# Lightbrite88/Argon_Monte_Carlo

Hardware: AMD Instinct MI355X
Metric: particle-steps/sec (higher is better)
Workload: dtype f64; 1 GPU; cube_1e5; geometry=cube, n_particles=100000, n_per_gpu=100000, parallelism=single GPU

## Files before the change

### argon_monte_carlo_amd/csrc/amc_grid.hip

```cpp
#include <stdlib.h>

#include "amc_grid_dev.h"

#define AMC_CR2_INFLATE (1.0 + 1.0e-9)

__global__ __launch_bounds__(256) void k_bin_lists(const double *__restrict__ x, const double *__restrict__ y,
                                                   const double *__restrict__ z, long long n, amc_grid G, amc_lists B,
                                                   amc_dev_counters *cnt, amc_ovl V)
{
    const long long p = (long long)blockIdx.x * blockDim.x + threadIdx.x;
    if (p >= n) return;
    if (V.skip_epoch && (unsigned int)(V.adj_head[p] >> 32) == V.skip_epoch) return;
    bool outside = false;
    amc_list_insert(G, B, (int)p, x[p], y[p], z[p], &outside);
    if (outside) atomicOr(&cnt->flags, 8ULL);
}

struct amc_adj {
    unsigned long long *head;
    int4 *rec;
    int4 *sd;
    int4 *sl_meta;
    int *sl_hits, *ev_gen;
    unsigned int epoch;
    unsigned long long *mark;
};

AMC_DEV int amc_push_candidate(int a, int b, int max_cand, amc_dev_counters *cnt, const amc_adj &D)
{
    const unsigned int k = atomicAdd(&cnt->cand_count, 1u);
    if (k < (unsigned)max_cand) {
        const int hi = a > b ? a : b, lo = a > b ? b : a;
        int4 r;
        r.x = hi; r.y = lo; r.z = -1; r.w = -1;
        if (D.head) {
            const unsigned long long mine = ((unsigned long long)D.epoch << 32) | (unsigned long long)k;
            const unsigned long long oi = atomicExch(&D.head[hi], mine), oj = atomicExch(&D.head[lo], mine);
            r.z = ((unsigned int)(oi >> 32) == D.epoch) ? (int)(unsigned int)(oi & 0xffffffffULL) : -1;
            r.w = ((unsigned int)(oj >> 32) == D.epoch) ? (int)(unsigned int)(oj & 0xffffffffULL) : -1;
            auto mark = [&](int kd) {
                const unsigned long long old = atomicExch(&D.mark[kd], mine);
                if ((unsigned int)(old >> 32) == D.epoch) D.mark[kd] = ((unsigned long long)D.epoch << 32) | AMC_MARK_MULTI;
            };
            if (r.z >= 0) mark(r.z);
            if (r.w >= 0) mark(r.w);
        }
        D.rec[k] = r;
        D.sd[k] = make_int4(-1, -1, 0, 0);
        if (D.head) {
            D.sl_meta[2 * k] = make_int4(-1, 2 * (int)k, 0, 0);
            D.sl_meta[2 * k + 1] = make_int4(-1, 2 * (int)k + 1, 0, 0);
            atomicAnd(&D.sl_hits[2 * k], 0);
            atomicAnd(&D.sl_hits[2 * k + 1], 0);
            *(int4 *)&D.ev_gen[4 * k] = make_int4(0, 0, 0, 0);
        }
        return (int)k;
    }
    atomicOr(&cnt->flags, 1ULL);
    return -1;
}

AMC_DEV void amc_detect_node(const amc_grid &G, const amc_lists &B, int node, double cr2i, double cr_probe, int max_cand,
                             amc_dev_counters *cnt, const amc_adj &D, const int *od_stall = nullptr, int od_tick = 0)
{
    const int stalled = od_stall ? *od_stall : 0;
    amc_rec me_r = B.rec[node];
    const int live = (B.node_of && node < B.n) ? B.node_of[node] : node;
    if (stalled && od_tick > stalled) return;
    if (me_r.x != me_r.x) {
        if (live == node) return;
        node = live;
        me_r = B.rec[node];
        if (me_r.x != me_r.x) return;
    }
    const int me_p = amc_node_particle(B, node);
    double3 me;
    amc_rec_pos(G, me_r, me.x, me.y, me.z);
    auto found_pair = [&](int q) { amc_push_candidate(me_p, amc_node_particle(B, q), max_cand, cnt, D); };
    int q[9];
    q[0] = amc_rec_next(me_r);
    {
        int ocx, ocy, ocz;
        amc_grid_coords(G, me.x, me.y, me.z, ocx, ocy, ocz);
        const int c_own = amc_grid_cell(G, ocx, ocy, ocz, nullptr);
        int c_lo[4], c_hi[4];
        const int nc = amc_grid_box_ranges(G, me.x, me.y, me.z, cr_probe, c_lo, c_hi);
        int cell[8];
#pragma unroll
        for (int k = 0; k < 4; k++)
#pragma unroll
            for (int t = 0; t < 2; t++) {
                const int c = c_lo[k < nc ? k : 0] + t;
                cell[2 * k + t] = (k < nc && c <= c_hi[k < nc ? k : 0] && c < c_own) ? c : -1;
            }
        unsigned long long hv[8];
#pragma unroll
        for (int e = 0; e < 8; e++) hv[e] = (cell[e] >= 0) ? B.head[cell[e]] : 0ULL;
#pragma unroll
        for (int e = 0; e < 8; e++)
            q[1 + e] = (cell[e] >= 0 && (unsigned int)(hv[e] >> 32) == B.epoch) ? (int)(unsigned int)(hv[e] & 0xffffffffULL) : -1;
    }
    for (;;) {
        bool live = false;
#pragma unroll
        for (int e = 0; e < 9; e++) live |= q[e] >= 0;
        if (!live) break;
        amc_rec o[9];
#pragma unroll
        for (int e = 0; e < 9; e++)
            if (q[e] >= 0) o[e] = B.rec[q[e]];
#pragma unroll
        for (int e = 0; e < 9; e++)
            if (q[e] >= 0) {
                double ox, oy, oz;
                amc_rec_pos(G, o[e], ox, oy, oz);
                const double ex = ox - me.x, ey = oy - me.y, ez = oz - me.z;
                if (ex * ex + ey * ey + ez * ez < cr2i) found_pair(q[e]);
                q[e] = amc_rec_next(o[e]);
            }
    }
}

#ifndef AMC_DETECT_MINW
#define AMC_DETECT_MINW 4
#endif
__global__ __launch_bounds__(256, AMC_DETECT_MINW) void k_detect_lists(amc_grid G, amc_lists B, long long n, double cr2i, double cr_probe,
                                                      int max_cand, amc_dev_counters *cnt, amc_adj D, const int *extra_count,
                                                      int max_extra, const int *od_stall, int od_tick, int *wctl_rearm)
{
    const long long nb = (n + blockDim.x - 1) / blockDim.x;
    if ((long long)blockIdx.x < nb) {
        const long long p = (long long)blockIdx.x * blockDim.x + threadIdx.x;
        if (p < n) amc_detect_node(G, B, (int)p, cr2i, cr_probe, max_cand, cnt, D, od_stall, od_tick);
        if (wctl_rearm && p == 0 && !(*od_stall && od_tick > *od_stall)) {
            amc_resolve_ctl *wc = (amc_resolve_ctl *)wctl_rearm;
            for (int b = 0; b < 16; b++) wctl_rearm[32 + b] = 0;
            wc->nslots = 0; wc->nhist = 0; wc->nedges = 0; wc->nfp = 0; wc->ovf = 0; wc->dirty = 0; wc->nclusters = 0;
            wc->changed = 0; wc->active = 0; wc->cur_round = 1;
        }
        return;
    }
    if (!extra_count) return;
    int ne = *extra_count;
    if (ne > max_extra) ne = max_extra;
    const int stride = (int)((gridDim.x - nb) * blockDim.x);
    for (int e = (int)((blockIdx.x - nb) * blockDim.x + threadIdx.x); e < ne; e += stride)
        amc_detect_node(G, B, (int)n + e, cr2i, cr_probe, max_cand, cnt, D, od_stall, od_tick);
}

__global__ __launch_bounds__(256) void k_detect_own(amc_grid G, amc_lists B, long long lo, long long hi, double cr2i,
                                                    double cr_probe, int *__restrict__ out, int cap, amc_dev_counters *cnt)
{
    const long long p = lo + (long long)blockIdx.x * blockDim.x + threadIdx.x;
    if (p >= hi) return;
    amc_rec me_r = B.rec[p];
    const int live = B.node_of ? B.node_of[p] : (int)p;
    if (me_r.x != me_r.x) {
        if (live == (int)p) return;
        me_r = B.rec[live];
        if (me_r.x != me_r.x) return;
    }
    double3 me;
    amc_rec_pos(G, me_r, me.x, me.y, me.z);
    int c_lo[4], c_hi[4];
    const int nc = amc_grid_box_ranges(G, me.x, me.y, me.z, cr_probe, c_lo, c_hi);
    int q[8];
    unsigned long long hv[8];
#pragma unroll
    for (int k = 0; k < 4; k++)
#pragma unroll
        for (int t = 0; t < 2; t++) {
            const int c = c_lo[k < nc ? k : 0] + t;
            const bool on = k < nc && c <= c_hi[k < nc ? k : 0];
            hv[2 * k + t] = on ? B.head[c] : 0ULL;
            q[2 * k + t] = on ? 0 : -1;
        }
#pragma unroll
    for (int e = 0; e < 8; e++)
        q[e] = (q[e] == 0 && (unsigned int)(hv[e] >> 32) == B.epoch) ? (int)(unsigned int)(hv[e] & 0xffffffffULL) : -1;
    for (;;) {
        bool live = false;
#pragma unroll
        for (int e = 0; e < 8; e++) live |= q[e] >= 0;
        if (!live) break;
        amc_rec o[8];
#pragma unroll
        for (int e = 0; e < 8; e++)
            if (q[e] >= 0) o[e] = B.rec[q[e]];
#pragma unroll
        for (int e = 0; e < 8; e++)
            if (q[e] >= 0) {
                double ox, oy, oz;
                amc_rec_pos(G, o[e], ox, oy, oz);
                const double ex = ox - me.x, ey = oy - me.y, ez = oz - me.z;
                const int pq = amc_node_particle(B, q[e]);
                if (pq < (int)p && ex * ex + ey * ey + ez * ez < cr2i) {
                    const int k = atomicAdd(&out[0], 1);
                    if (k < cap) { out[2 + 2 * k] = (int)p; out[3 + 2 * k] = pq; }
                    else atomicOr(&cnt->flags, 1ULL);
                }
                q[e] = amc_rec_next(o[e]);
            }
    }
}

__global__ __launch_bounds__(256) void k_ingest_candidates(const int *__restrict__ blocks, int world, int block_ints, int cap,
                                                           int max_cand, amc_dev_counters *cnt, amc_adj D, int *__restrict__ own)
{
    const int gtid = blockIdx.x * blockDim.x + threadIdx.x, gstride = gridDim.x * blockDim.x;
    for (int r = 0; r < world; r++) {
        const int *b = blocks + (size_t)r * block_ints;
        int nr = b[0];
        if (nr > cap) {
            nr = cap;
            if (gtid == 0) atomicOr(&cnt->flags, 1ULL);
        }
        for (int k = gtid; k < nr; k += gstride) amc_push_candidate(b[2 + 2 * k], b[3 + 2 * k], max_cand, cnt, D);
    }
    if (gtid == 0) own[0] = 0;
}

#define AP_T 256
__global__ __launch_bounds__(AP_T) void k_detect_allpairs(const double *__restrict__ x, const double *__restrict__ y,
                                                          const double *__restrict__ z, int n, int ntiles, double cr2i,
                                                          int max_cand, amc_dev_counters *cnt, amc_adj D)
{
    int bi = (int)((sqrt(8.0 * (double)blockIdx.x + 1.0) - 1.0) * 0.5);
    while ((long long)(bi + 1) * (bi + 2) / 2 <= (long long)blockIdx.x) bi++;
    while ((long long)bi * (bi + 1) / 2 > (long long)blockIdx.x) bi--;
    const int bj = (int)(blockIdx.x - (long long)bi * (bi + 1) / 2);
    if (bi >= ntiles) return;
    __shared__ double tx[AP_T], ty[AP_T], tz[AP_T];
    const int j0 = bj * AP_T;
    const int jj = j0 + threadIdx.x;
    tx[threadIdx.x] = (jj < n) ? x[jj] : 0.0;
    ty[threadIdx.x] = (jj < n) ? y[jj] : 0.0;
    tz[threadIdx.x] = (jj < n) ? z[jj] : 0.0;
    __syncthreads();
    const int i = bi * AP_T + threadIdx.x;
    if (i >= n) return;
    const double xi = x[i], yi = y[i], zi = z[i];
    int jmax = n - j0;
    if (jmax > AP_T) jmax = AP_T;
    if (bi == bj && jmax > (int)threadIdx.x) jmax = threadIdx.x;
#pragma unroll 4
    for (int k = 0; k < jmax; k++) {
        const double ex = tx[k] - xi, ey = ty[k] - yi, ez = tz[k] - zi;
        const double d2 = fma(ez, ez, fma(ey, ey, ex * ex));
        if (d2 < cr2i) amc_push_candidate(i, j0 + k, max_cand, cnt, D);
    }
}

hipError_t amc_launch_bin(amc_ctx *c)
{
    if (c->allpairs || c->n <= 0) return hipSuccess;
    const long long n = c->n;
    c->B.epoch++;
    c->step.lists_age = -1;
    amc_prof_begin(c, AMC_K_BIN_COUNT);
    amc_ovl V;
    V.adj_head = nullptr; V.skip_epoch = 0;
    AMC_LAUNCH(c, k_bin_lists, dim3((unsigned)((n + 255) / 256)), dim3(256), c->S.x, c->S.y, c->S.z, n,
                       c->G, c->B, c->d_cnt, V);
    amc_prof_end(c);
    return hipGetLastError();
}

hipError_t amc_launch_bin_ovl(amc_ctx *c, int to, unsigned int skip_epoch, hipStream_t stream)
{
    const long long n = c->n;
    amc_ovl V;
    V.adj_head = c->W.adj_head; V.skip_epoch = skip_epoch;
    amc_prof_begin(c, AMC_K_BIN_COUNT);
    AMC_LAUNCH_ON(c, stream, k_bin_lists, dim3((unsigned)((n + 255) / 256)), dim3(256), c->S_buf[to].x, c->S_buf[to].y, c->S_buf[to].z, n,
                  c->G, c->B_buf[to], c->d_cnt, V);
    amc_prof_end(c);
    return hipGetLastError();
}

#define AP2_T 1024
#define AP2_R 4
#define AP2_THREADS (AP2_T / AP2_R)
#define AP2_CHUNK 8
__global__ __launch_bounds__(AP2_THREADS) void k_detect_allpairs_tiled(const double *__restrict__ x, const double *__restrict__ y,
                                                               const double *__restrict__ z, int n, int ntiles, double thr,
                                                               double ox, double oy, double oz,
                                                               int max_cand, amc_dev_counters *cnt, amc_adj D)
{
    int bi = (int)((sqrt(8.0 * (double)blockIdx.x + 1.0) - 1.0) * 0.5);
    while ((long long)(bi + 1) * (bi + 2) / 2 <= (long long)blockIdx.x) bi++;
    while ((long long)bi * (bi + 1) / 2 > (long long)blockIdx.x) bi--;
    const int bj = (int)(blockIdx.x - (long long)bi * (bi + 1) / 2);
    if (bi >= ntiles) return;
    __shared__ double tx[AP2_T], ty[AP2_T], tz[AP2_T], tn[AP2_T];
    const int j0 = bj * AP2_T;
    for (int t = threadIdx.x; t < AP2_T; t += AP2_THREADS) {
        const int jj = j0 + t;
        const bool in = jj < n;
        const double X = in ? x[jj] - ox : 0.0, Y = in ? y[jj] - oy : 0.0, Z = in ? z[jj] - oz : 0.0;
        tx[t] = X; ty[t] = Y; tz[t] = Z;
        tn[t] = in ? fma(Z, Z, fma(Y, Y, X * X)) : 1.0e300;
    }
    __syncthreads();
    int ii[AP2_R];
    double ax[AP2_R], ay[AP2_R], az[AP2_R], ti[AP2_R];
#pragma unroll
    for (int r = 0; r < AP2_R; r++) {
        ii[r] = bi * AP2_T + r * AP2_THREADS + (int)threadIdx.x;
        const bool in = ii[r] < n;
        const double X = in ? x[ii[r]] - ox : 0.0, Y = in ? y[ii[r]] - oy : 0.0, Z = in ? z[ii[r]] - oz : 0.0;
        ax[r] = -2.0 * X; ay[r] = -2.0 * Y; az[r] = -2.0 * Z;
        ti[r] = in ? thr - fma(Z, Z, fma(Y, Y, X * X)) : -1.0e300;
    }
    const bool diag = bi == bj;
    for (int k0 = 0; k0 < AP2_T; k0 += AP2_CHUNK) {
        bool any = false;
#pragma unroll
        for (int u = 0; u < AP2_CHUNK; u++) {
            const double jx = tx[k0 + u], jy = ty[k0 + u], jz = tz[k0 + u], jn = tn[k0 + u];
#pragma unroll
            for (int r = 0; r < AP2_R; r++) any |= fma(az[r], jz, fma(ay[r], jy, fma(ax[r], jx, jn))) < ti[r];
        }
        if (any) {
            for (int u = 0; u < AP2_CHUNK; u++) {
                const int j = j0 + k0 + u;
                const double jx = tx[k0 + u], jy = ty[k0 + u], jz = tz[k0 + u], jn = tn[k0 + u];
#pragma unroll
                for (int r = 0; r < AP2_R; r++)
                    if (fma(az[r], jz, fma(ay[r], jy, fma(ax[r], jx, jn))) < ti[r] && (diag ? j < ii[r] : true))
                        amc_push_candidate(ii[r], j, max_cand, cnt, D);
            }
        }
    }
}

static unsigned int next_sweep_epoch(unsigned int epoch)
{
    epoch = (epoch + 1u) & 0x3fffffffu;
    return epoch ? epoch : 1u;
}

hipError_t amc_launch_detect(amc_ctx *c)
{
    const long long n = c->n;
    if (n <= 0) return hipSuccess;
    const double cr2i = c->allpairs || c->detect_ap ? c->P.collision_range * c->P.collision_range * AMC_CR2_INFLATE : c->G.cr2_probe;
    amc_adj D;
    c->step.sweep_epoch = next_sweep_epoch(c->step.sweep_epoch);
    c->step.plan_split = !c->allpairs && !(c->h_host_ncand && *c->h_host_ncand <= c->plan_small);
    D.head = c->allpairs ? nullptr : c->W.adj_head; D.rec = c->W.cand4; D.sd = c->W.cand_s; D.epoch = c->step.sweep_epoch;
    D.sl_meta = c->W.sl_meta; D.sl_hits = c->W.sl_hits; D.ev_gen = c->W.ev_gen; D.mark = c->W.cand_mark;
    amc_prof_begin(c, AMC_K_DETECT);
    if (c->detect_ap) {
        if (n >= 16 * AP2_T && c->G.ncells > 0) {
            const int ntiles = (int)((n + AP2_T - 1) / AP2_T);
            const long long nblocks = (long long)ntiles * (ntiles + 1) / 2;
            const double ex = c->G.gx * c->G.h, ey = c->G.gy * c->G.h, ez = c->G.gz * c->G.h;
            const double thr = cr2i + 64.0 * 1.1102230246251565e-16 * (ex * ex + ey * ey + ez * ez);
            AMC_LAUNCH(c, k_detect_allpairs_tiled, dim3((unsigned)nblocks), dim3(AP2_THREADS), c->S.x, c->S.y,
                               c->S.z, (int)n, ntiles, thr, c->G.x0, c->G.y0, c->G.z0, c->W.max_cand, c->d_cnt, D);
        } else {
            const int ntiles = (int)((n + AP_T - 1) / AP_T);
            const long long nblocks = (long long)ntiles * (ntiles + 1) / 2;
            if (nblocks > 0)
                AMC_LAUNCH(c, k_detect_allpairs, dim3((unsigned)nblocks), dim3(AP_T), c->S.x, c->S.y,
                                   c->S.z, (int)n, ntiles, cr2i, c->W.max_cand, c->d_cnt, D);
        }
    } else {
        const bool extras = c->B.extra != nullptr && c->keep_K < 2;
        const int slot = (c->B.extra == c->extra_buf[1]) ? 1 : 0;
        const int bs = c->detect_bs;
        AMC_LAUNCH(c, k_detect_lists, dim3((unsigned)((n + bs - 1) / bs) + (extras ? 4u : 0u)), dim3(bs), c->G, c->B, n, cr2i,
                   c->G.cr_probe, c->W.max_cand, c->d_cnt, D, (const int *)(extras ? c->extra_count + slot : nullptr),
                   c->max_extra, (const int *)(c->od_active ? c->d_od : nullptr), c->od_tick,
                   (c->od_active && !c->step.od_prev_ordered) ? c->W.wctl : nullptr);
    }
    amc_prof_end(c);
    return hipGetLastError();
}

hipError_t amc_launch_detect_own(amc_ctx *c)
{
    const long long cnt = c->hi - c->lo;
    amc_prof_begin(c, AMC_K_DETECT);
    if (cnt > 0)
        AMC_LAUNCH(c, k_detect_own, dim3((unsigned)((cnt + 255) / 256)), dim3(256), c->G, c->B, (long long)c->lo, (long long)c->hi,
                   c->G.cr2_probe, c->G.cr_probe, c->MG.cand_send, c->MG.cand_cap, c->d_cnt);
    amc_prof_end(c);
    return hipGetLastError();
}

hipError_t amc_launch_ingest(amc_ctx *c, int world)
{
    amc_adj D;
    c->step.sweep_epoch = next_sweep_epoch(c->step.sweep_epoch);
    c->step.plan_split = !(c->h_host_ncand && *c->h_host_ncand <= c->plan_small);
    D.head = c->W.adj_head; D.rec = c->W.cand4; D.sd = c->W.cand_s; D.epoch = c->step.sweep_epoch;
    D.sl_meta = c->W.sl_meta; D.sl_hits = c->W.sl_hits; D.ev_gen = c->W.ev_gen; D.mark = c->W.cand_mark;
    amc_prof_begin(c, AMC_K_DETECT);
    AMC_LAUNCH(c, k_ingest_candidates, dim3(16), dim3(256), (const int *)c->MG.cand_recv, world, 2 + 2 * c->MG.cand_cap, c->MG.cand_cap,
               c->W.max_cand, c->d_cnt, D, c->MG.cand_send);
    amc_prof_end(c);
    return hipGetLastError();
}
```

### argon_monte_carlo_amd/csrc/amc_internal.h

```cpp
#pragma once
#include <hip/hip_runtime.h>
#include <hip/hip_ext.h>
#include <stdint.h>

#include <string>
#include <vector>

#include "amc_device.h"

#define RS_SLOT_DOUBLES 12

struct amc_state {
    double *x, *y, *z, *vx, *vy, *vz, *d, *dx, *dy, *dz;
    double *px, *py, *pz;
    uint8_t *flag;
};

struct amc_grid {
    double x0, y0, z0, h;
    double inv_h;
    int uniform;
    int gx, gy, gz;
    int ncells;
    double cr_probe;
    double cr2_probe;
    const int *lay_lo;
    const int *lay_n;
    const int *lay_off;
};

struct amc_rec {
    float x, y, z;
    int next;
};
#define AMC_MARK_MULTI 0xffffffffu
struct amc_lists {
    unsigned long long *head;
    amc_rec *rec;
    unsigned int epoch;
    int n;
    int *extra;
    int *cell_of;
    int *node_of;
    int *wave_count;
    int wave_cap;
};
#define AMC_LIST_KEEP_DEFAULT_PORE 4
#define AMC_EXTRA_NODES(n) ((int)std::min<long long>(std::max<long long>(4096, (long long)(n) / 64), 1 << 22))

struct amc_ovl {
    const unsigned long long *adj_head;
    unsigned int skip_epoch;
};

struct amc_lazy {
    int *slot_of;
    const double *state;
    const uint8_t *moved;
    int enabled;
};

struct amc_resolve_ctl {
    int nslots, nedges, nhist, nev, dirty, changed, nhits, nfp, ovf, nclusters, ncomplex;
    int rounds, ncand, active, ok, edges_done;
    int lazy_ns, nslots0, hist_begin, cur_round;
};
struct rs_event {
    int phase, i, j, which;
    long long cell;
    int slot, pad;
    double val[4];
};
struct amc_resolve_ws {
    int4 *cand4, *cand_s;
    unsigned long long *cand_mark;
    int max_cand;
    unsigned long long *adj_head;
    int *slot_of;
    unsigned int *victim;
    int max_slots;
    int4 *sl_meta;
    int *sl_hits;
    uint8_t *sl_moved;
    double *sl_state;
    int *edge_a, *edge_b;
    int max_edges;
    double4 *hist;
    int max_hist;
    int *ov_head, *ov_next;
    int *ev_gen;
    rs_event *ev;
    int *ctl;
    int *wctl;
    int *raise_dev, *raise_host;
    int raise_tick;
    int *sl_label, *sl_tmp;
    uint8_t *sl_dirty;
    unsigned long long *sl_key;
    int *order;
    double *cw_d[10];
    int *cw_tmp, *cw_pidx, *cw_slot;
    uint8_t *cw_flag, *cw_moved;
};

struct amc_temp_handover {
    int hits_case = -1, hits_n = 0;
    int ahead_case = -1;
    std::vector<int> perm;
    int parked_case = -1, parked_n = 0;
    std::vector<int> parked_perm;
    void fresh() { hits_case = ahead_case = parked_case = -1; hits_n = parked_n = 0; perm.clear(); parked_perm.clear(); }
};

struct amc_temp_ws {
    int *idx, *count;
    double *t, *contact, *normal, *dir, *Es, *dpz, *dE;
    unsigned char *ok;
    int *h_idx, *h_count;
    double *h_contact, *h_normal, *h_dir, *h_Es, *h_dpz, *h_dE;
    void *pin;
    int cap;
    int *def_idx;
    double *def_dir, *def_Es, *def_dpz, *def_dE;
    double *h_def_Es, *h_def_dpz, *h_def_dE;
    amc_temp_handover h;
};

struct temp_dev_segments {
    int *idx, *count;
    double *t, *contact, *normal, *dir, *Es, *dpz, *dE;
    unsigned char *ok;
    int cap;
};
struct amc_temp_pass {
    amc_temp_rng g;
    temp_dev_segments D;
};
struct amc_temp_row {
    double sums[3];
    unsigned int had;
    unsigned int pad;
};
struct amc_temp_dev_ws {
    temp_dev_segments seg;
    amc_temp_row *series;
    int64_t series_cap, series_n;
    int *perm;
    int *ovf;
    amc_temp_pass *pass;
    bool fetched;
    int h_count[7];
    std::vector<int> h_idx[7];
    std::vector<double> h_dpz[7], h_dE[7];
    std::vector<unsigned char> h_ok[7];
};

struct amc_fields_grid_dev {
    int kind, n1, n2, n3, bins;
    double lo[3], hi[3], w[3];
};

// ... 251 lines not shown
```

### argon_monte_carlo_amd/csrc/amc_stream.hip

```cpp
#include <stdlib.h>
#include <string.h>

#include <algorithm>

#include "amc_commit_dev.h"
#include "amc_energised_dev.h"

struct amc_stream_counts {
    int nwall, nerr, noob, noob_pre;
};

template <int GEOM>
AMC_DEV void amc_stream_particle(amc_particle &q, const amc_params &P, const amc_out &O, double dt, int stages, int ip,
                                 double &px, double &py, double &pz, amc_stream_counts &cn)
{
    if ((stages & AMC_ST_BOUNDS_PRE) && GEOM != AMC_GEOM_CUBE)
        cn.noob_pre = amc_bounds(P, q.x, q.y, q.z, GEOM == AMC_GEOM_PORE_ENERGISED);
    if (stages & AMC_ST_DRIFT) {
        px = q.x; py = q.y; pz = q.z;
        const double sx = dt * q.vx, sy = dt * q.vy, sz = dt * q.vz;
        q.x += sx; q.y += sy; q.z += sz;
        q.d += fabs(sqrt(sx * sx + sy * sy + sz * sz));
        q.dx += fabs(sx); q.dy += fabs(sy); q.dz += fabs(sz);
    }
    if (stages & AMC_ST_WALLS) {
        if (GEOM == AMC_GEOM_CUBE) {
#define AMC_CUBE_AXIS(pos, vel, W)                                                                    \
    if (pos > W) { const double t_ = (pos - W) / vel; vel = -vel; pos = W + t_ * vel; }                \
    if (pos < 0) { const double t_ = pos / vel; vel = -vel; pos = t_ * vel; }
            AMC_CUBE_AXIS(q.x, q.vx, P.cube_x)
            AMC_CUBE_AXIS(q.y, q.vy, P.cube_y)
            AMC_CUBE_AXIS(q.z, q.vz, P.cube_z)
#undef AMC_CUBE_AXIS
        } else if (GEOM == AMC_GEOM_PORE) {
            const double zb = P.z_gap_bottom, zt = P.z_gap_top;
            const double r0 = sqrt(px * px + py * py);
            if (sqrt(q.x * q.x + q.y * q.y) > P.R_oa) {
                if (amc_side_wall(q, P.R_oa_c, true, O, 1, ip)) cn.nerr++; else cn.nwall++;
            }
            if (q.z < 0) { amc_vertical_wall(q, 0.0, O, 2, ip); cn.nwall++; }
            if (q.z > P.H) { amc_vertical_wall(q, P.H, O, 3, ip); cn.nwall++; }
            if ((pz > P.z_cold) && (q.z < P.z_cold) && (sqrt(q.x * q.x + q.y * q.y) > P.R_p)) {
                amc_vertical_wall(q, P.z_cold, O, 4, ip); cn.nwall++;
            }
            if ((pz < P.h_oa) && (q.z > P.h_oa) && (sqrt(q.x * q.x + q.y * q.y) > P.R_p)) {
                amc_vertical_wall(q, P.h_oa, O, 5, ip); cn.nwall++;
            }
            if ((pz < zt) && (pz > zb) && (r0 < P.R_g) && (sqrt(q.x * q.x + q.y * q.y) > P.R_g)) {
                if (amc_side_wall(q, P.R_g_c, true, O, 6, ip)) cn.nerr++; else cn.nwall++;
            }
            if ((r0 > P.R_p) && (q.z < zb) && (pz < zt) && (pz > zb)) {
                amc_vertical_wall(q, zb, O, 7, ip); cn.nwall++;
            }
            if ((r0 > P.R_p) && (q.z > zt) && (pz < zt) && (pz > zb)) {
                amc_vertical_wall(q, zt, O, 8, ip); cn.nwall++;
            }
            if ((r0 < P.R_p) && (sqrt(q.x * q.x + q.y * q.y) > P.R_p) &&
                (((q.z < P.z_cold) && (q.z > zt)) || ((q.z < zb) && (q.z > P.h_oa)))) {
                if (amc_side_wall(q, P.R_p_c, true, O, 9, ip)) cn.nerr++; else cn.nwall++;
            }
        } else if (GEOM == AMC_GEOM_PORE_ENERGISED) {
            if (sqrt(q.x * q.x + q.y * q.y) > P.R_oa) {
                if (amc_side_wall(q, P.R_oa_c, false, O, 1, ip)) cn.nerr++;
            }
            if (q.z < 0) { const double t_ = (q.z - 0.0) / q.vz; q.vz = -q.vz; q.z = 0.0 + t_ * q.vz; }
            if (q.z > P.H) { const double t_ = (q.z - P.H) / q.vz; q.vz = -q.vz; q.z = P.H + t_ * q.vz; }
        }
    }
    if ((stages & AMC_ST_BOUNDS) && GEOM != AMC_GEOM_CUBE)
        cn.noob = amc_bounds(P, q.x, q.y, q.z, GEOM == AMC_GEOM_PORE_ENERGISED);
}

AMC_DEV void amc_stream_count(const amc_out &O, const amc_stream_counts &cn, int bounds_slot, int ip)
{
    if (!(cn.nwall | cn.nerr | cn.noob | cn.noob_pre)) return;
    if (O.wev.count) {
        amc_wev_rec r;
        r.p = ip; r.kind = 1; r.a = cn.nwall | (cn.nerr << 16); r.b = cn.noob | (cn.noob_pre << 16);
        r.v[0] = r.v[1] = r.v[2] = r.v[3] = 0.0;
        amc_wev_append(O, r);
        return;
    }
    if (cn.nwall) atomicAdd(&O.banks[amc_bank_id()].n_wall, (unsigned long long)cn.nwall);
    if (cn.nerr) atomicAdd(&O.banks[amc_bank_id()].n_fp_errors, (unsigned long long)cn.nerr);
    if (cn.noob) atomicAdd(bounds_slot ? &O.cnt->n_oob_pp : &O.cnt->n_oob_walls, (unsigned long long)cn.noob);
    if (cn.noob_pre) atomicAdd(&O.cnt->n_oob_pp, (unsigned long long)cn.noob_pre);
}

#define AMC_LD(p) __builtin_nontemporal_load(&(p))
#define AMC_ST(p, v) __builtin_nontemporal_store((v), &(p))

template <int GEOM, int TEMP = 0>
__global__ __launch_bounds__(256) void k_stream(amc_state S, amc_state S_out, amc_params P, amc_out O, double dt, int stages,
                                                long long lo, long long hi, int keep_prior, int bounds_slot,
                                                amc_grid G, amc_lists B, int build_lists, amc_lazy L, amc_commit_args C,
                                                amc_ovl V, const amc_temp_pass *TP)
{
    const int stalled = C.od_stall ? *C.od_stall : 0;
    if (C.enabled) {
        const unsigned nstream = gridDim.x - (unsigned)C.enabled;
        if (blockIdx.x >= nstream) {
            if (stalled && C.od_tick > stalled) return;
            amc_out Oc = O;
            Oc.step = C.step;
            amc_commit_part(C, Oc, G, S, (int)((blockIdx.x - nstream) * blockDim.x + threadIdx.x), (int)(C.enabled * blockDim.x));
            return;
        }
    }
    const long long p = lo + (long long)blockIdx.x * blockDim.x + threadIdx.x;
    if (p >= hi) return;
    if (V.skip_epoch && (unsigned int)(V.adj_head[p] >> 32) == V.skip_epoch) return;
    const int wave_id = (int)(blockIdx.x * (blockDim.x >> 6) + (threadIdx.x >> 6));
    const int keep_count0 = build_lists == 3 ? B.wave_count[wave_id] : 0;
    const int keep_cell = build_lists == 3 ? B.cell_of[p] : -1, keep_node = build_lists == 3 ? B.node_of[p] : (int)p;
    amc_particle q;
    q.x = AMC_LD(S.x[p]); q.y = AMC_LD(S.y[p]); q.z = AMC_LD(S.z[p]);
    q.vx = AMC_LD(S.vx[p]); q.vy = AMC_LD(S.vy[p]); q.vz = AMC_LD(S.vz[p]);
    const double x_in = q.x, y_in = q.y, z_in = q.z, vx_in = q.vx, vy_in = q.vy, vz_in = q.vz;
    const bool need_acc = (stages & (AMC_ST_DRIFT | AMC_ST_WALLS)) != 0;
    bool flag_in = false;
    double d_in = 0, dx_in = 0, dy_in = 0, dz_in = 0;
    q.d = q.dx = q.dy = q.dz = 0; q.flag = false;
    if (need_acc) {
        q.d = AMC_LD(S.d[p]); q.dx = AMC_LD(S.dx[p]); q.dy = AMC_LD(S.dy[p]); q.dz = AMC_LD(S.dz[p]);
        q.flag = S.flag[p] != 0;
        flag_in = q.flag; d_in = q.d; dx_in = q.dx; dy_in = q.dy; dz_in = q.dz;
    }
    if (stalled && C.od_tick > stalled) return;
    bool force = S_out.x != S.x;
    if (L.enabled) {
        const int sl = L.slot_of[p];
        if (sl >= 0) {
            L.slot_of[p] = -1;
            if (L.moved[sl]) {
                const double *t = L.state + (size_t)sl * RS_SLOT_DOUBLES;
                q.x = t[0]; q.y = t[1]; q.z = t[2]; q.vx = t[3]; q.vy = t[4]; q.vz = t[5];
                q.d = t[6]; q.dx = t[7]; q.dy = t[8]; q.dz = t[9]; q.flag = t[10] != 0.0;
                force = true;
            }
        }
    }
    const bool wr_acc = need_acc || force;
    double px = q.x, py = q.y, pz = q.z;
    if (!(stages & AMC_ST_DRIFT) && GEOM != AMC_GEOM_CUBE && (stages & AMC_ST_WALLS)) { px = S.px[p]; py = S.py[p]; pz = S.pz[p]; }
    amc_stream_counts cn = {0, 0, 0, 0};
    const bool temp_cases = GEOM == AMC_GEOM_PORE_ENERGISED && TEMP != 0;
    amc_stream_particle<GEOM>(q, P, O, dt, temp_cases ? (stages & ~AMC_ST_BOUNDS) : stages, (int)p, px, py, pz, cn);
    if ((stages & AMC_ST_DRIFT) && keep_prior && GEOM != AMC_GEOM_CUBE) { S.px[p] = px; S.py[p] = py; S.pz[p] = pz; }
    if (GEOM == AMC_GEOM_PORE_ENERGISED && TEMP != 0) {
        if (temp_any_mask(P, q.x, q.y, q.z, px, py, pz)) {
            temp_particle t;
            t.x = q.x; t.y = q.y; t.z = q.z; t.vx = q.vx; t.vy = q.vy; t.vz = q.vz;
            t.d = q.d; t.dx = q.dx; t.dy = q.dy; t.dz = q.dz; t.flag = q.flag ? 1 : 0; t.nwall = 0; t.nerr = 0;
            temp_cases_particle<true>(P, O, TP->g, (unsigned int)O.step, TP->D, (int)p, px, py, pz, t);
            q.x = t.x; q.y = t.y; q.z = t.z; q.vx = t.vx; q.vy = t.vy; q.vz = t.vz;
            q.d = t.d; q.dx = t.dx; q.dy = t.dy; q.dz = t.dz; q.flag = t.flag != 0;
            cn.nwall += t.nwall; cn.nerr += t.nerr;
        }
        if (stages & AMC_ST_BOUNDS) cn.noob = amc_bounds(P, q.x, q.y, q.z, true);
    }

    if (force || q.x != x_in) AMC_ST(S_out.x[p], q.x);
    if (force || q.y != y_in) AMC_ST(S_out.y[p], q.y);
    if (force || q.z != z_in) AMC_ST(S_out.z[p], q.z);
    if (force || q.vx != vx_in) S_out.vx[p] = q.vx;
    if (force || q.vy != vy_in) S_out.vy[p] = q.vy;
    if (force || q.vz != vz_in) S_out.vz[p] = q.vz;
    if (wr_acc) {
        if (force || q.d != d_in) AMC_ST(S_out.d[p], q.d);
        if (force || q.dx != dx_in) AMC_ST(S_out.dx[p], q.dx);
        if (force || q.dy != dy_in) AMC_ST(S_out.dy[p], q.dy);
        if (force || q.dz != dz_in) AMC_ST(S_out.dz[p], q.dz);
        if (force || q.flag != flag_in) S_out.flag[p] = q.flag ? 1 : 0;
    }
    if (build_lists == 1) {
        bool outside = false;
        amc_list_insert(G, B, (int)p, q.x, q.y, q.z, &outside);
        if (outside) atomicOr(&O.cnt->flags, 8ULL);
    } else if (build_lists) {
        bool outside = false, overflow = false;
        const int nc = amc_list_keep(G, B, (int)p, q.x, q.y, q.z, build_lists == 2, wave_id, keep_count0, keep_cell, keep_node, &outside, &overflow);
        if ((int)__lane_id() == __ffsll((long long)__ballot(true)) - 1) B.wave_count[wave_id] = nc;
        if (outside) atomicOr(&O.cnt->flags, 8ULL);
        if (overflow) atomicOr(&O.cnt->flags, 1ULL);
    }
    amc_stream_count(O, cn, bounds_slot, (int)p);
}

struct amc_fixup_args {
    amc_state S_in, S_out;
    amc_lists B;
    int *extra;
    int *extra_count;
    int max_extra;
    const unsigned long long *adj_head;
    const unsigned int *victim;
    unsigned int sweep_epoch;
    amc_wev wev;
    unsigned int *wev_clear;
    int *extra_clear;
    int stages, step_sweep, step_stream;
    double dt;
};

#define AMC_FIXUP_SLOT_BLOCKS 24

template <int GEOM>
__global__ __launch_bounds__(256) void k_fixup(amc_fixup_args F, amc_params P, amc_out O, amc_grid G, amc_commit_args C)
{
    if (blockIdx.x == 0 && threadIdx.x < AMC_COUNTER_BANKS) F.wev_clear[threadIdx.x] = 0;
    if (blockIdx.x == 0 && threadIdx.x == 0) *F.extra_clear = 0;
    if (F.sweep_epoch && blockIdx.x < AMC_FIXUP_SLOT_BLOCKS) {
        const int gtid = blockIdx.x * blockDim.x + threadIdx.x, gstride = AMC_FIXUP_SLOT_BLOCKS * blockDim.x;
        amc_resolve_ctl *ctl = C.ctl;
        const bool active = ctl->active != 0;
        const bool ok = ctl->ok && !ctl->ovf;
        const int ns = !active ? 0 : (ctl->nslots < C.max_slots ? ctl->nslots : C.max_slots);
        amc_out Od = O;
        Od.wev.count = nullptr;
        Od.step = F.step_stream;
        for (int s = gtid; s < ns; s += gstride) {
            const int p = C.sl_meta[s].x;
            if (p < 0) continue;
            amc_particle q;
            if (ok && C.sl_moved[s]) {
                const double *t = C.sl_state + (size_t)s * RS_SLOT_DOUBLES;
                q.x = t[0]; q.y = t[1]; q.z = t[2]; q.vx = t[3]; q.vy = t[4]; q.vz = t[5];
                q.d = t[6]; q.dx = t[7]; q.dy = t[8]; q.dz = t[9]; q.flag = t[10] != 0.0;
            } else {
                q.x = F.S_in.x[p]; q.y = F.S_in.y[p]; q.z = F.S_in.z[p]; q.vx = F.S_in.vx[p]; q.vy = F.S_in.vy[p]; q.vz = F.S_in.vz[p];
                q.d = F.S_in.d[p]; q.dx = F.S_in.dx[p]; q.dy = F.S_in.dy[p]; q.dz = F.S_in.dz[p]; q.flag = F.S_in.flag[p] != 0;
            }
            const bool marked = (unsigned int)(F.adj_head[p] >> 32) == F.sweep_epoch;
            double px = q.x, py = q.y, pz = q.z;
            amc_stream_counts cn = {0, 0, 0, 0};
            amc_stream_particle<GEOM>(q, P, Od, F.dt, F.stages, p, px, py, pz, cn);
            F.S_out.x[p] = q.x; F.S_out.y[p] = q.y; F.S_out.z[p] = q.z;
            F.S_out.vx[p] = q.vx; F.S_out.vy[p] = q.vy; F.S_out.vz[p] = q.vz;
            F.S_out.d[p] = q.d; F.S_out.dx[p] = q.dx; F.S_out.dy[p] = q.dy; F.S_out.dz[p] = q.dz; F.S_out.flag[p] = q.flag ? 1 : 0;
            bool outside = false;
            if (marked) {
                amc_list_insert(G, F.B, p, q.x, q.y, q.z, &outside);
            } else {
                ((float *)&F.B.rec[p])[0] = __int_as_float(0x7fc00000);
                const int e = atomicAdd(F.extra_count, 1);
                atomicAdd(&O.cnt->n_refiled, 1);
                if (e < F.max_extra) {
                    F.extra[e] = p;
                    amc_list_insert(G, F.B, F.B.n + e, q.x, q.y, q.z, &outside);
                } else {
                    atomicOr(&O.cnt->flags, 4ULL);
                }
            }
            if (outside) atomicOr(&O.cnt->flags, 8ULL);
            C.slot_of[p] = -1;
            amc_stream_count(Od, cn, 0, p);
        }
    } else if (F.sweep_epoch) {
        amc_out Os = O;
        Os.wev.count = nullptr;
        Os.step = F.step_sweep;
        amc_commit_part(C, Os, G, F.S_in, (int)((blockIdx.x - AMC_FIXUP_SLOT_BLOCKS) * blockDim.x + threadIdx.x),
                        (int)((gridDim.x - AMC_FIXUP_SLOT_BLOCKS) * blockDim.x));
    }
    amc_out Od = O;
    Od.wev.count = nullptr;
    Od.step = F.step_stream;
    for (int b = blockIdx.x; b < AMC_COUNTER_BANKS; b += gridDim.x) {
        unsigned int nb = F.wev.count[b];
        if (nb > (unsigned)F.wev.cap) nb = (unsigned)F.wev.cap;
        for (unsigned int k = threadIdx.x; k < nb; k += blockDim.x) {
            const amc_wev_rec r = F.wev.rec[(size_t)b * F.wev.cap + k];
            if (F.sweep_epoch && F.victim[r.p] == F.sweep_epoch) continue;
            if (r.kind == 0) {
                amc_emit(Od, r.a, 0, r.p, -1, 0, r.v[0], r.v[1], r.v[2], r.v[3]);
            } else {
                amc_stream_counts cn = {r.a & 0xffff, r.a >> 16, r.b & 0xffff, r.b >> 16};
                amc_stream_count(Od, cn, 0, r.p);
            }
        }
    }
}

amc_commit_args amc_make_commit_args(amc_ctx *c)
{
    const amc_resolve_ws &W = c->W;
    amc_commit_args C;
    C.ctl = (amc_resolve_ctl *)W.ctl; C.hist = W.hist; C.ov_head = W.ov_head; C.ev_gen = W.ev_gen; C.ev = W.ev;
    C.sl_meta = W.sl_meta; C.sl_hits = W.sl_hits; C.sl_moved = W.sl_moved; C.sl_state = W.sl_state; C.slot_of = W.slot_of;
    C.max_slots = W.max_slots; C.max_hist = W.max_hist; C.lo = c->lo; C.hi = c->hi; C.count_pp = c->MG.count_pp ? 1 : 0;
    C.defer = c->step.commit_defer ? 1 : 0; C.nogrid = c->allpairs ? 1 : 0; C.enabled = 0;
    C.step = c->step.commit_step;
    C.od_stall = nullptr; C.od_tick = 0; C.from_wide = 0; C.wctl = nullptr; C.host_ncand = nullptr;
    return C;
}

int amc_list_build_mode(amc_ctx *c, int owner, bool kept)
{
    amc_step_state &T = c->step;
    if (!kept) { c->B.epoch++; T.lists_age = -1; return 1; }
    if (T.lists_owner != owner) T.lists_age = -1;
    T.lists_owner = owner;
    if (T.lists_age < 0 || T.lists_age + 1 >= c->keep_K) { c->B.epoch++; T.lists_age = 0; T.full_builds++; return 2; }
    T.lists_age++;
    return 3;
}

static void launch_k_stream(amc_ctx *c, hipStream_t stream, unsigned blocks, int threads, const amc_state &S, const amc_state &S_out,
                            const amc_out &O, double dt, int stages, long long lo, long long hi, int keep_prior, int bounds_slot,
                            const amc_lists &B, int build, const amc_lazy &L, const amc_commit_args &C, const amc_ovl &V)
{
    const bool cases = (stages & AMC_ST_TEMP_CASES) != 0;
    auto *k = k_stream<AMC_GEOM_CUBE>;
    switch (c->P.geometry) {
    case AMC_GEOM_CUBE: break;
    case AMC_GEOM_PORE: k = k_stream<AMC_GEOM_PORE>; break;
    case AMC_GEOM_PORE_ENERGISED: k = cases ? k_stream<AMC_GEOM_PORE_ENERGISED, 1> : k_stream<AMC_GEOM_PORE_ENERGISED>; break;
    default: return;
    }
    AMC_LAUNCH_ON(c, stream, k, dim3(blocks), dim3(threads), S, S_out, c->P, O, dt, stages, lo, hi, keep_prior, bounds_slot, c->G, B,
                  build, L, C, V, (const amc_temp_pass *)(cases ? c->TD.pass : nullptr));
}

hipError_t amc_launch_stream(amc_ctx *c, double dt, int stages, int bounds_slot, bool fuse_bin)
{
    const int threads = c->stream_bs;
    int build = 0;
    if (fuse_bin && !c->allpairs && c->lo == 0 && c->hi == c->n) build = amc_list_build_mode(c, 1, c->keep_K >= 2 && c->B.cell_of);
    amc_lazy L;
    memset(&L, 0, sizeof L);
    if (c->step.lazy_pending) {
        const amc_resolve_ws &W = c->W;
        L.slot_of = W.slot_of; L.state = W.sl_state; L.moved = W.sl_moved;
        L.enabled = 1;
        c->step.lazy_pending = false;
    }
    const long long cnt = c->hi - c->lo;
    if (cnt <= 0) return hipSuccess;
    amc_commit_args C = amc_make_commit_args(c);
    const amc_resolve_ws &W_ = c->W;
    unsigned extra = 0;
    if (c->step.commit_pending) {
        const long long lag = c->h_host_ncand ? *c->h_host_ncand : 0;
        extra = (unsigned)std::min<long long>(std::max<long long>((2 * lag + 255) / 256, 4), AMC_COMMIT_BLOCKS);
        C.enabled = (int)extra;
        c->step.commit_pending = false;
        if (c->od_active && !c->step.od_prev_ordered) { C.from_wide = 1; C.wctl = W_.wctl; C.host_ncand = c->d_host_ncand; }
    }
    if (c->od_active) { C.od_stall = c->d_od; C.od_tick = c->od_tick; }
    const unsigned blocks = (unsigned)((cnt + threads - 1) / threads) + extra;
    const int kp = (stages & AMC_ST_TEMP_CASES) ? (int)(c->P.reserved0 & 1) : (c->keep_prior ? 1 : 0);
    amc_ovl V;
    V.adj_head = nullptr; V.skip_epoch = 0;
    if ((stages & AMC_ST_TEMP_CASES) && (c->P.geometry != AMC_GEOM_PORE_ENERGISED || !c->TD.pass)) return hipErrorInvalidValue;
    amc_prof_begin(c, (stages == AMC_ST_BOUNDS) ? AMC_K_BOUNDS : AMC_K_DRIFT_WALLS);
    launch_k_stream(c, c->stream, blocks, threads, c->S, c->S, c->out, dt, stages, c->lo, c->hi, kp, bounds_slot, c->B, build, L, C, V);
    amc_prof_end(c);
    return hipGetLastError();
}

hipError_t amc_launch_stream_ovl(amc_ctx *c, double dt, int stages, int from, unsigned int skip_epoch, hipStream_t stream,
                                 bool build_lists)
{
    const int to = 1 - from;
    amc_lists &Bn = c->B_buf[to];
    Bn.epoch++;
    c->step.lists_age = -1;
    amc_lazy L;
    memset(&L, 0, sizeof L);
    amc_commit_args C = amc_make_commit_args(c);
    amc_ovl V;
    V.adj_head = c->W.adj_head; V.skip_epoch = skip_epoch;
    amc_out O = c->out;
    O.wev = c->wev_buf[c->out.step & 1];
    const unsigned blocks = (unsigned)((c->n + 255) / 256);
    amc_prof_begin(c, AMC_K_DRIFT_WALLS);
    launch_k_stream(c, stream, blocks, 256, c->S_buf[from], c->S_buf[to], O, dt, stages, 0, c->n, 0, 0, Bn, build_lists ? 1 : 0, L, C, V);
    amc_prof_end(c);
    return hipGetLastError();
}

hipError_t amc_launch_fixup(amc_ctx *c, double dt, int stages, int from, unsigned int sweep_epoch)
{
    const int to = 1 - from;
    amc_fixup_args F;
    F.S_in = c->S_buf[from]; F.S_out = c->S_buf[to];
    F.B = c->B_buf[to];
    F.extra = c->extra_buf[to]; F.extra_count = c->extra_count + to; F.max_extra = c->max_extra;
    F.adj_head = c->W.adj_head; F.victim = c->W.victim; F.sweep_epoch = sweep_epoch;
    F.wev = c->wev_buf[c->out.step & 1];
    F.wev_clear = c->wev_buf[1 - (c->out.step & 1)].count;
    F.extra_clear = c->extra_count + from;
    F.stages = stages; F.step_stream = c->out.step; F.step_sweep = c->out.step - 1; F.dt = dt;
    amc_commit_args C = amc_make_commit_args(c);
    C.defer = 1;
    C.enabled = 1;
    amc_prof_begin(c, AMC_K_FIXUP);
    if (c->P.geometry == AMC_GEOM_CUBE)
        AMC_LAUNCH(c, k_fixup<AMC_GEOM_CUBE>, dim3(AMC_COMMIT_BLOCKS), dim3(256), F, c->P, c->out, c->G, C);
    else
        AMC_LAUNCH(c, k_fixup<AMC_GEOM_PORE>, dim3(AMC_COMMIT_BLOCKS), dim3(256), F, c->P, c->out, c->G, C);
    amc_prof_end(c);
    return hipGetLastError();
}
```

Baseline: 2.379 billion particle-steps/s.

## Pack hot kernel arguments into 64-byte records read with wide scalar loads

Both the detect and stream kernels now receive a packed record of their hot arguments, placed at the start of the kernarg segment and fetched with a few 16-dword scalar loads. Pointers are cast to the global address space so the compiler can emit global rather than flat memory ops. The od_stall read is routed through a VGPR index, and the S_out comparison becomes a precomputed flag. The aim is lower kernel prologue latency and cheaper addressing, at the cost of fragile layout assumptions enforced by static_asserts and inline asm constraints.

After: 2.353 billion particle-steps/s. -1.1%, worse.

```diff
diff --git a/argon_monte_carlo_amd/csrc/amc_grid.hip b/argon_monte_carlo_amd/csrc/amc_grid.hip
--- a/argon_monte_carlo_amd/csrc/amc_grid.hip
+++ b/argon_monte_carlo_amd/csrc/amc_grid.hip
@@ -1,4 +1,6 @@
+#include <stddef.h>
 #include <stdlib.h>
+#include <string.h>
 
 #include "amc_grid_dev.h"
 
@@ -63,7 +65,12 @@
 AMC_DEV void amc_detect_node(const amc_grid &G, const amc_lists &B, int node, double cr2i, double cr_probe, int max_cand,
                              amc_dev_counters *cnt, const amc_adj &D, const int *od_stall = nullptr, int od_tick = 0)
 {
-    const int stalled = od_stall ? *od_stall : 0;
+    int stalled = 0;
+    if (od_stall) {
+        int lane_zero;
+        asm("v_mov_b32 %0, 0" : "=v"(lane_zero));
+        stalled = od_stall[lane_zero];
+    }
     amc_rec me_r = B.rec[node];
     const int live = (B.node_of && node < B.n) ? B.node_of[node] : node;
     if (stalled && od_tick > stalled) return;
@@ -124,14 +131,59 @@
 #ifndef AMC_DETECT_MINW
 #define AMC_DETECT_MINW 4
 #endif
-__global__ __launch_bounds__(256, AMC_DETECT_MINW) void k_detect_lists(amc_grid G, amc_lists B, long long n, double cr2i, double cr_probe,
-                                                      int max_cand, amc_dev_counters *cnt, amc_adj D, const int *extra_count,
-                                                      int max_extra, const int *od_stall, int od_tick, int *wctl_rearm)
-{
-    const long long nb = (n + blockDim.x - 1) / blockDim.x;
-    if ((long long)blockIdx.x < nb) {
-        const long long p = (long long)blockIdx.x * blockDim.x + threadIdx.x;
-        if (p < n) amc_detect_node(G, B, (int)p, cr2i, cr_probe, max_cand, cnt, D, od_stall, od_tick);
+struct amc_detect_args {
+    amc_grid G;
+    amc_lists B;
+    long long n;
+    double cr2i, cr_probe;
+    int max_cand;
+    unsigned bs;
+    amc_dev_counters *cnt;
+    const int *od_stall;
+    int od_tick;
+    unsigned nb;
+    unsigned long long *d_head;
+    int4 *d_rec;
+    unsigned long long *d_mark;
+    unsigned int d_epoch;
+    int pad0;
+    int4 *d_sd, *d_sl_meta;
+    int *d_sl_hits, *d_ev_gen;
+    const int *extra_count;
+    int *wctl_rearm;
+    int max_extra;
+    int pad1[3];
+};
+#define AMC_DETECT_ARG_LOADS 4
+static_assert(sizeof(amc_detect_args) == (AMC_DETECT_ARG_LOADS + 1) * 64 && offsetof(amc_detect_args, d_sd) == AMC_DETECT_ARG_LOADS * 64,
+              "the head of the argument record is read as four 16-dword scalar loads");
+
+__global__ __launch_bounds__(256, AMC_DETECT_MINW) void k_detect_lists(amc_detect_args A_in_kernarg)
+{
+    const __attribute__((address_space(4))) amc_v16i *arg_src =
+        (const __attribute__((address_space(4))) amc_v16i *)__builtin_amdgcn_kernarg_segment_ptr();
+    amc_v16i arg_w[AMC_DETECT_ARG_LOADS];
+#pragma unroll
+    for (int j = 0; j < AMC_DETECT_ARG_LOADS; j++) arg_w[j] = arg_src[j];
+    asm("" : "+s"(arg_w[0]), "+s"(arg_w[1]), "+s"(arg_w[2]), "+s"(arg_w[3]));
+    amc_detect_args A = A_in_kernarg;
+    __builtin_memcpy(&A, arg_w, sizeof arg_w);
+    amc_grid &G = A.G; amc_lists &B = A.B;
+    G.lay_lo = AMC_GP(G.lay_lo); G.lay_n = AMC_GP(G.lay_n); G.lay_off = AMC_GP(G.lay_off);
+    B.head = AMC_GP(B.head); B.rec = AMC_GP(B.rec); B.extra = AMC_GP(B.extra); B.cell_of = AMC_GP(B.cell_of);
+    B.node_of = AMC_GP(B.node_of); B.wave_count = AMC_GP(B.wave_count);
+    amc_adj D;
+    D.head = AMC_GP(A.d_head); D.rec = AMC_GP(A.d_rec); D.mark = AMC_GP(A.d_mark); D.epoch = A.d_epoch;
+    D.sd = A.d_sd; D.sl_meta = A.d_sl_meta; D.sl_hits = A.d_sl_hits; D.ev_gen = A.d_ev_gen;
+    amc_dev_counters *cnt = AMC_GP(A.cnt);
+    const int *extra_count = A.extra_count, *od_stall = AMC_GP(A.od_stall);
+    int *wctl_rearm = A.wctl_rearm;
+    const long long n = A.n;
+    const unsigned nb = A.nb, bs = A.bs;
+    const int od_tick = A.od_tick, max_cand = A.max_cand;
+    if (blockIdx.x < nb) {
+        const long long p = (long long)blockIdx.x * bs + threadIdx.x;
+        if (p < n) amc_detect_node(G, B, (int)p, A.cr2i, A.cr_probe, max_cand, cnt, D, od_stall, od_tick);
         if (wctl_rearm && p == 0 && !(*od_stall && od_tick > *od_stall)) {
             amc_resolve_ctl *wc = (amc_resolve_ctl *)wctl_rearm;
             for (int b = 0; b < 16; b++) wctl_rearm[32 + b] = 0;
@@ -142,10 +194,10 @@
     }
     if (!extra_count) return;
     int ne = *extra_count;
-    if (ne > max_extra) ne = max_extra;
-    const int stride = (int)((gridDim.x - nb) * blockDim.x);
-    for (int e = (int)((blockIdx.x - nb) * blockDim.x + threadIdx.x); e < ne; e += stride)
-        amc_detect_node(G, B, (int)n + e, cr2i, cr_probe, max_cand, cnt, D, od_stall, od_tick);
+    if (ne > A.max_extra) ne = A.max_extra;
+    const int stride = (int)((gridDim.x - nb) * bs);
+    for (int e = (int)((blockIdx.x - nb) * bs + threadIdx.x); e < ne; e += stride)
+        amc_detect_node(G, B, (int)n + e, A.cr2i, A.cr_probe, max_cand, cnt, D, od_stall, od_tick);
 }
 
 __global__ __launch_bounds__(256) void k_detect_own(amc_grid G, amc_lists B, long long lo, long long hi, double cr2i,
@@ -370,10 +422,16 @@
         const bool extras = c->B.extra != nullptr && c->keep_K < 2;
         const int slot = (c->B.extra == c->extra_buf[1]) ? 1 : 0;
         const int bs = c->detect_bs;
-        AMC_LAUNCH(c, k_detect_lists, dim3((unsigned)((n + bs - 1) / bs) + (extras ? 4u : 0u)), dim3(bs), c->G, c->B, n, cr2i,
-                   c->G.cr_probe, c->W.max_cand, c->d_cnt, D, (const int *)(extras ? c->extra_count + slot : nullptr),
-                   c->max_extra, (const int *)(c->od_active ? c->d_od : nullptr), c->od_tick,
-                   (c->od_active && !c->step.od_prev_ordered) ? c->W.wctl : nullptr);
+        amc_detect_args A;
+        memset(&A, 0, sizeof A);
+        A.G = c->G; A.B = c->B; A.n = n; A.cr2i = cr2i; A.cr_probe = c->G.cr_probe; A.max_cand = c->W.max_cand; A.cnt = c->d_cnt;
+        A.d_head = D.head; A.d_rec = D.rec; A.d_mark = D.mark; A.d_epoch = D.epoch;
+        A.d_sd = D.sd; A.d_sl_meta = D.sl_meta; A.d_sl_hits = D.sl_hits; A.d_ev_gen = D.ev_gen;
+        A.extra_count = extras ? c->extra_count + slot : nullptr; A.max_extra = c->max_extra;
+        A.od_stall = c->od_active ? c->d_od : nullptr; A.od_tick = c->od_tick;
+        A.wctl_rearm = (c->od_active && !c->step.od_prev_ordered) ? c->W.wctl : nullptr;
+        A.bs = (unsigned)bs; A.nb = (unsigned)((n + bs - 1) / bs);
+        AMC_LAUNCH(c, k_detect_lists, dim3(A.nb + (extras ? 4u : 0u)), dim3(bs), A);
     }
     amc_prof_end(c);
     return hipGetLastError();
diff --git a/argon_monte_carlo_amd/csrc/amc_internal.h b/argon_monte_carlo_amd/csrc/amc_internal.h
--- a/argon_monte_carlo_amd/csrc/amc_internal.h
+++ b/argon_monte_carlo_amd/csrc/amc_internal.h
@@ -7,6 +7,9 @@
 #include <vector>
 
 #include "amc_device.h"
+
+typedef int amc_v16i __attribute__((ext_vector_type(16)));
+#define AMC_GP(p) ((decltype(p))(__attribute__((address_space(1))) void *)(unsigned long long)(p))
 
 #define RS_SLOT_DOUBLES 12
 
diff --git a/argon_monte_carlo_amd/csrc/amc_stream.hip b/argon_monte_carlo_amd/csrc/amc_stream.hip
--- a/argon_monte_carlo_amd/csrc/amc_stream.hip
+++ b/argon_monte_carlo_amd/csrc/amc_stream.hip
@@ -1,3 +1,4 @@
+#include <assert.h>
 #include <stdlib.h>
 #include <string.h>
 
@@ -89,33 +90,104 @@
 
 #define AMC_LD(p) __builtin_nontemporal_load(&(p))
 #define AMC_ST(p, v) __builtin_nontemporal_store((v), &(p))
+struct amc_stream_hot {
+    double *x, *y, *z, *vx, *vy, *vz, *d, *dx, *dy, *dz;
+    uint8_t *flag;
+    int out_differs;
+    int stages;
+    long long lo, hi;
+    const int *od_stall;
+    int od_tick;
+    unsigned nstream;
+    unsigned int skip_epoch;
+    int lazy_enabled;
+    const unsigned long long *adj_head;
+    int *slot_of;
+    const uint8_t *moved;
+    const double *state;
+    double dt;
+    union {
+        struct { double cube_x, cube_y, cube_z; };
+        struct { int *cell_of, *node_of, *wave_count; };
+    };
+    double gx0, gy0, gz0, inv_h;
+    int gx, gy, gz;
+    unsigned block_size;
+    int build_lists;
+    unsigned int epoch;
+    unsigned long long *head;
+    amc_rec *rec;
+    int bounds_slot, keep_prior;
+    amc_dev_counters *cnt;
+    amc_counter_bank *banks;
+    unsigned int *wev_count;
+    const int *lay;
+    int pad[2];
+};
+#define AMC_HOT_LOADS 5
+static_assert(sizeof(amc_stream_hot) == AMC_HOT_LOADS * 64, "the hot record is read as five 16-dword scalar loads");
 
 template <int GEOM, int TEMP = 0>
-__global__ __launch_bounds__(256) void k_stream(amc_state S, amc_state S_out, amc_params P, amc_out O, double dt, int stages,
-                                                long long lo, long long hi, int keep_prior, int bounds_slot,
+__global__ __launch_bounds__(256) void k_stream(amc_stream_hot H_in_kernarg, amc_state S, amc_state S_out, amc_params P, amc_out O,
+                                                double dt, int stages, long long lo, long long hi, int keep_prior, int bounds_slot,
                                                 amc_grid G, amc_lists B, int build_lists, amc_lazy L, amc_commit_args C,
                                                 amc_ovl V, const amc_temp_pass *TP)
 {
-    const int stalled = C.od_stall ? *C.od_stall : 0;
-    if (C.enabled) {
-        const unsigned nstream = gridDim.x - (unsigned)C.enabled;
-        if (blockIdx.x >= nstream) {
-            if (stalled && C.od_tick > stalled) return;
-            amc_out Oc = O;
-            Oc.step = C.step;
-            amc_commit_part(C, Oc, G, S, (int)((blockIdx.x - nstream) * blockDim.x + threadIdx.x), (int)(C.enabled * blockDim.x));
-            return;
-        }
-    }
-    const long long p = lo + (long long)blockIdx.x * blockDim.x + threadIdx.x;
+    amc_stream_hot H = H_in_kernarg;
+    if (GEOM == AMC_GEOM_CUBE) {
+        const __attribute__((address_space(4))) amc_v16i *hot_src =
+            (const __attribute__((address_space(4))) amc_v16i *)__builtin_amdgcn_kernarg_segment_ptr();
+        amc_v16i hot_w[AMC_HOT_LOADS];
+#pragma unroll
+        for (int j = 0; j < AMC_HOT_LOADS; j++) hot_w[j] = hot_src[j];
+        asm volatile("" : "+s"(hot_w[0]), "+s"(hot_w[1]), "+s"(hot_w[2]), "+s"(hot_w[3]), "+s"(hot_w[4]));
+        __builtin_memcpy(&H, hot_w, sizeof H);
+    }
+    S.x = AMC_GP(H.x); S.y = AMC_GP(H.y); S.z = AMC_GP(H.z); S.vx = AMC_GP(H.vx); S.vy = AMC_GP(H.vy); S.vz = AMC_GP(H.vz);
+    S.d = AMC_GP(H.d); S.dx = AMC_GP(H.dx); S.dy = AMC_GP(H.dy); S.dz = AMC_GP(H.dz); S.flag = AMC_GP(H.flag);
+    const bool out_differs = H.out_differs != 0;
+    stages = H.stages; lo = H.lo; hi = H.hi; dt = H.dt; keep_prior = H.keep_prior; bounds_slot = H.bounds_slot;
+    C.od_stall = AMC_GP(H.od_stall); C.od_tick = H.od_tick;
+    V.skip_epoch = H.skip_epoch; V.adj_head = AMC_GP(H.adj_head);
+    L.enabled = H.lazy_enabled; L.slot_of = AMC_GP(H.slot_of); L.moved = AMC_GP(H.moved); L.state = AMC_GP(H.state);
+    if (GEOM == AMC_GEOM_CUBE) { P.cube_x = H.cube_x; P.cube_y = H.cube_y; P.cube_z = H.cube_z; }
+    else { B.cell_of = AMC_GP(H.cell_of); B.node_of = AMC_GP(H.node_of); B.wave_count = AMC_GP(H.wave_count); }
+    G.x0 = H.gx0; G.y0 = H.gy0; G.z0 = H.gz0; G.inv_h = H.inv_h; G.gx = H.gx; G.gy = H.gy; G.gz = H.gz;
+    G.uniform = GEOM == AMC_GEOM_CUBE ? 1 : 0;
+    if (GEOM != AMC_GEOM_CUBE) { G.lay_lo = AMC_GP(H.lay); G.lay_n = G.lay_lo + H.gz; G.lay_off = G.lay_lo + 2 * H.gz; }
+    B.head = AMC_GP(H.head); B.rec = AMC_GP(H.rec); B.epoch = H.epoch; build_lists = H.build_lists;
+    O.cnt = AMC_GP(H.cnt); O.banks = AMC_GP(H.banks); O.wev.count = AMC_GP(H.wev_count);
+    const unsigned block_size = H.block_size;
+    if (blockIdx.x >= H.nstream) {
+        const int stalled = H.od_stall ? *(const __attribute__((address_space(4))) int *)(unsigned long long)H.od_stall : 0;
+        if (stalled && C.od_tick > stalled) return;
+        amc_out Oc = O;
+        Oc.step = C.step;
+        amc_commit_part(C, Oc, G, S, (int)((blockIdx.x - H.nstream) * block_size + threadIdx.x), (int)(C.enabled * block_size));
+        return;
+    }
+    const long long p = lo + (long long)blockIdx.x * block_size + threadIdx.x;
     if (p >= hi) return;
     if (V.skip_epoch && (unsigned int)(V.adj_head[p] >> 32) == V.skip_epoch) return;
-    const int wave_id = (int)(blockIdx.x * (blockDim.x >> 6) + (threadIdx.x >> 6));
-    const int keep_count0 = build_lists == 3 ? B.wave_count[wave_id] : 0;
-    const int keep_cell = build_lists == 3 ? B.cell_of[p] : -1, keep_node = build_lists == 3 ? B.node_of[p] : (int)p;
+    const int wave_id = (int)(blockIdx.x * (block_size >> 6) + (threadIdx.x >> 6));
+    int keep_count0 = 0, keep_cell = -1, keep_node = (int)p;
+    if (build_lists == 3) {
+        if (GEOM == AMC_GEOM_CUBE) {
+            asm volatile("" : "+s"(B.wave_count), "+s"(B.cell_of), "+s"(B.node_of));
+            B.wave_count = AMC_GP(B.wave_count); B.cell_of = AMC_GP(B.cell_of); B.node_of = AMC_GP(B.node_of);
+        }
+        keep_count0 = B.wave_count[wave_id]; keep_cell = B.cell_of[p]; keep_node = B.node_of[p];
+    }
+    int stalled = 0;
+    if (C.od_stall) {
+        int lane_zero;
+        asm("v_mov_b32 %0, 0" : "=v"(lane_zero));
+        stalled = C.od_stall[lane_zero];
+    }
     amc_particle q;
     q.x = AMC_LD(S.x[p]); q.y = AMC_LD(S.y[p]); q.z = AMC_LD(S.z[p]);
     q.vx = AMC_LD(S.vx[p]); q.vy = AMC_LD(S.vy[p]); q.vz = AMC_LD(S.vz[p]);
+    const int slot_word = L.enabled ? L.slot_of[p] : -1;
     const double x_in = q.x, y_in = q.y, z_in = q.z, vx_in = q.vx, vy_in = q.vy, vz_in = q.vz;
     const bool need_acc = (stages & (AMC_ST_DRIFT | AMC_ST_WALLS)) != 0;
     bool flag_in = false;
@@ -127,9 +199,19 @@
         flag_in = q.flag; d_in = q.d; dx_in = q.dx; dy_in = q.dy; dz_in = q.dz;
     }
     if (stalled && C.od_tick > stalled) return;
-    bool force = S_out.x != S.x;
+    bool force = out_differs;
+    if (out_differs) {
+        asm volatile("" : "+s"(S_out.x), "+s"(S_out.y), "+s"(S_out.z), "+s"(S_out.vx), "+s"(S_out.vy), "+s"(S_out.vz));
+        asm volatile("" : "+s"(S_out.d), "+s"(S_out.dx), "+s"(S_out.dy), "+s"(S_out.dz), "+s"(S_out.flag));
+        S_out.x = AMC_GP(S_out.x); S_out.y = AMC_GP(S_out.y); S_out.z = AMC_GP(S_out.z);
+        S_out.vx = AMC_GP(S_out.vx); S_out.vy = AMC_GP(S_out.vy); S_out.vz = AMC_GP(S_out.vz);
+        S_out.d = AMC_GP(S_out.d); S_out.dx = AMC_GP(S_out.dx); S_out.dy = AMC_GP(S_out.dy); S_out.dz = AMC_GP(S_out.dz);
+        S_out.flag = AMC_GP(S_out.flag);
+    } else {
+        S_out = S;
+    }
     if (L.enabled) {
-        const int sl = L.slot_of[p];
+        const int sl = slot_word;
         if (sl >= 0) {
             L.slot_of[p] = -1;
             if (L.moved[sl]) {
@@ -318,7 +400,23 @@
     case AMC_GEOM_PORE_ENERGISED: k = cases ? k_stream<AMC_GEOM_PORE_ENERGISED, 1> : k_stream<AMC_GEOM_PORE_ENERGISED>; break;
     default: return;
     }
-    AMC_LAUNCH_ON(c, stream, k, dim3(blocks), dim3(threads), S, S_out, c->P, O, dt, stages, lo, hi, keep_prior, bounds_slot, c->G, B,
+    const amc_grid &G = c->G;
+    amc_stream_hot H;
+    memset(&H, 0, sizeof H);
+    H.x = S.x; H.y = S.y; H.z = S.z; H.vx = S.vx; H.vy = S.vy; H.vz = S.vz; H.d = S.d; H.dx = S.dx; H.dy = S.dy; H.dz = S.dz;
+    H.flag = S.flag; H.out_differs = S_out.x != S.x ? 1 : 0;
+    H.stages = stages; H.lo = lo; H.hi = hi; H.dt = dt; H.keep_prior = keep_prior; H.bounds_slot = bounds_slot;
+    H.od_stall = C.od_stall; H.od_tick = C.od_tick; H.nstream = blocks - (unsigned)C.enabled;
+    H.skip_epoch = V.skip_epoch; H.adj_head = V.adj_head;
+    H.lazy_enabled = L.enabled; H.slot_of = L.slot_of; H.moved = L.moved; H.state = L.state;
+    if (c->P.geometry == AMC_GEOM_CUBE) { H.cube_x = c->P.cube_x; H.cube_y = c->P.cube_y; H.cube_z = c->P.cube_z; }
+    else { H.cell_of = B.cell_of; H.node_of = B.node_of; H.wave_count = B.wave_count; }
+    H.gx0 = G.x0; H.gy0 = G.y0; H.gz0 = G.z0; H.inv_h = G.inv_h; H.gx = G.gx; H.gy = G.gy; H.gz = G.gz; H.lay = G.lay_lo;
+    assert(c->allpairs || (G.uniform == (c->P.geometry == AMC_GEOM_CUBE ? 1 : 0) && G.lay_n == G.lay_lo + G.gz && G.lay_off == G.lay_lo + 2 * G.gz));
+    H.block_size = (unsigned)threads; H.build_lists = build;
+    H.head = B.head; H.rec = B.rec; H.epoch = B.epoch;
+    H.cnt = O.cnt; H.banks = O.banks; H.wev_count = O.wev.count;
+    AMC_LAUNCH_ON(c, stream, k, dim3(blocks), dim3(threads), H, S, S_out, c->P, O, dt, stages, lo, hi, keep_prior, bounds_slot, c->G, B,
                   build, L, C, V, (const amc_temp_pass *)(cases ? c->TD.pass : nullptr));
 }
 
```
